# Validation-m3sSAGE/GCN_Recommendation

Measured on AMD Instinct MI355X. Metric: propagated edges/sec (SpMM) + Recall@20, Amazon-Books 3-layer d=64, higher is better.
Workload: dtype f32; 1 GPU; C3 full Amazon-Books-2023 shape (10.3M users x 4.4M items x 29.5M interactions); generator=powerlaw, users=10300000, items=4400000, interactions=29500000, nnz=56305746, d=64, layers=3, brands=0, content_dim=0, hub_threshold=128, hub_mode=exact, emu_min_degree=1024, parallelism=single

## Files before the change

gcn_recommendation_amd/csrc/lgcn_engine.hip:

```cpp
#include "lgcn_kernels.h"

#include <string.h>
#include <algorithm>
#include <functional>
#include <new>
#include <vector>

namespace lgcn_detail {
int g_rows_per_group = 0;
int g_unroll = 0;
int g_mean_prefetch = 0;
int g_min_groups = 0;
int g_emu_margin = (128 << 4) | 4;
int g_sample_blocks = 0;
int g_fusion_bwd_blocks = 0;
}

namespace {
__global__ void k_coo_inspect(const int64_t* __restrict__ rows, const int64_t* __restrict__ cols,
                              int64_t nnz, int32_t n_rows, int32_t n_cols, int32_t* flags) {
    const int64_t j = (int64_t)blockIdx.x * blockDim.x + threadIdx.x;
    if (j >= nnz) return;
    const int64_t r = rows[j], c = cols[j];
    int f = 0;
// ... 964 lines not shown
    if (d < 1 || d > 2048 || n_hub_rows < 0) return LGCN_EINVAL;
    if (n_pre_rows < 0 || n_pre_rows > n_hub_rows) return LGCN_EINVAL;
    if (int e = check_epi(epi_host)) return e;
    if (n_hub_rows > 0 && (!hub_rows || !partials || !y || ldy < d)) return LGCN_EINVAL;
    return hub_combine(hub_rows, n_hub_rows, n_pre_rows, partials, y, ldy, d, *epi_host,
                       S(stream));
}

int lgcn_scale_rows(lgcn_rows_t x, int32_t n_rows, int32_t d, float div, float* y, int64_t ldy,
                    void* stream) {
    if (int e = valid_geom(n_rows, d)) return e;
    if (n_rows > 0 && (!y || ldy < d)) return LGCN_EINVAL;
    return scale_rows(x, n_rows, d, div, y, ldy, S(stream));
}

}

namespace {
constexpr int kPoolEvents = 1024;
struct EventPool {
    hipEvent_t ev[kPoolEvents];
    int n = 0;
    int next = 0;
    int32_t state[5] = {0, 0, 0, 0, 0};
};
struct StreamSet {
    hipStream_t aux[3];
    int n_aux;
};
struct Marks {
    hipEvent_t t0, t1;
    hipEvent_t* trace;
};
}

struct lgcn_sched {
    StreamSet lane0;
    EventPool* pool;
    int32_t slots[2];
    int chain;
    Marks marks;
    hipStream_t lane1_main;
    StreamSet lane1;
    hipEvent_t* trace_sides;
    hipEvent_t* timing_sides;
    int classes;
    int lk_normal;
// ... 57 lines not shown
                           static_cast<char*>(p.emu_meta) + b0 * d * LGCN_EMU_META_BYTES,
                           p.emu_stage ? p.emu_stage + b0 * (d + 1) * LGCN_EMU_BLOCK : nullptr,
                           live, s);
}

int part_walk(const lgcn_edge_t* edges, const lgcn_hub_plan_t& p, const EmuPart& q,
              const lgcn_rows_t& x, float xdiv, const uint32_t* x_nz, float* y, int64_t ldy,
              int32_t d, const lgcn_epilogue_t& ep, int slots, const lgcn_emu_row_t* live,
              hipStream_t s) {
    if (q.r1 <= q.r0) return 0;
    return lgcn_emu_walk(edges, p.emu_blocks, p.emu_rows + q.r0, q.r1 - q.r0, p.emu_rel,
                         p.emu_meta, p.emu_stage, x, xdiv, x_nz, y, ldy, d, &ep, slots,
                         live ? live + q.r0 : nullptr, s);
}

bool chain_ok(const lgcn_rows_t& x, int32_t d) {
    return lgcn_chain_supported(d) && x.ld % 4 == 0 && al16(x.p0) && al16(x.p1) && al16(x.p2);
}

int plan_layer(const int32_t* rowptr, const lgcn_edge_t* edges, const int32_t* row_ids,
               int32_t n, const lgcn_hub_plan_t& p, const lgcn_rows_t& x, float xdiv,
               const uint32_t* x_nz, float* y, int64_t ldy, int32_t d, const lgcn_epilogue_t& ep,
               const lgcn_sched* root, const StreamSet* ss, const Marks& mk, hipStream_t s,
               Deps* dp = nullptr) {
    const lgcn_sched* sc = ss ? root : nullptr;
    const int32_t ne = p.n_emu_rows;
    const bool live = x_nz && p.emu_live && ne > 0 && chain_ok(x, d) && (!sc || sc->chain);
    const bool chains = !live && ne > p.emu_part_rows[1] && chain_ok(x, d) && (!sc || sc->chain);
    if ((chains || live ? p.emu_part_blocks[1] : p.n_emu_blocks) > p.emu_scratch_blocks)
        return LGCN_EINVAL;
    hipEvent_t* tr = mk.trace;
    auto mark = [&](int k, hipStream_t st) -> int {
        return tr && tr[k] ? herr(hipEventRecord(tr[k], st)) : 0;
    };
    const EmuPart parts[3] = {{0, p.emu_part_rows[0], 0, p.emu_part_blocks[0]},
                              {p.emu_part_rows[0], p.emu_part_rows[1], p.emu_part_blocks[0],
                               p.emu_part_blocks[1]},
                              {p.emu_part_rows[1], ne, p.emu_part_blocks[1], p.n_emu_blocks}};
    const int slots[3] = {sc ? sc->slots[0] : 0, sc ? sc->slots[1] : 0, sc ? sc->slots[1] : 0};
    auto layer_kernel = [&](hipStream_t st) -> int {
        if (mk.t0)
            if (int e = herr(hipEventRecord(mk.t0, st))) return e;
        if (int e = spmm_layer(rowptr, edges, row_ids, n, p.threshold, p.items, p.n_items,
                               p.partials, x, y, ldy, d, ep, xdiv, x_nz, st))
            return e;
        if (mk.t1)
            if (int e = herr(hipEventRecord(mk.t1, st))) return e;
        return hub_combine(p.rows, p.n_rows, p.n_pre, p.partials, y, ldy, d, ep, st);
    };
    const bool has_late = dp && (dp->late[0] || dp->late[1] || dp->late[2] ||
                                 dp->late_emu[0] || dp->late_emu[1]);
    const bool defer_epi = sc && has_late && ep.mode == LGCN_EPI_MEAN && p.emu_out && ne > 0 &&
                           !live;
    lgcn_epilogue_t ep_rows;
    memset(&ep_rows, 0, sizeof(ep_rows));
    ep_rows.mode = LGCN_EPI_ROWS;
    auto emu_y = [&](int i) { return defer_epi ? p.emu_out + (int64_t)parts[i].r0 * d : y; };
    const int64_t emu_ld = defer_epi ? d : ldy;
    const lgcn_epilogue_t& emu_ep = defer_epi ? ep_rows : ep;
    auto chain_rows = [&](hipStream_t st) -> int {
        const EmuPart& q = parts[2];
        if (q.r1 <= q.r0) return 0;
        return lgcn_chain_rows(edges, p.emu_blocks, p.emu_rows + q.r0, q.r1 - q.r0, x, xdiv,
                               emu_y(2), emu_ld, d, &emu_ep, st);
    };
    const lgcn_emu_row_t* lflags =
        live ? lgcn_live_flags(p.emu_live, ne, p.n_emu_blocks) : nullptr;
    auto live_rows = [&](hipStream_t st) -> int {
        return lgcn_live_rows(edges, p.emu_blocks, p.n_emu_blocks, p.emu_rows, ne, x, xdiv, x_nz,
                              y, ldy, d, &ep, p.emu_part_rows[1], LGCN_LIVE_MAX, p.emu_live, st);
    };
    auto walked = [&](int i, hipStream_t st) -> int {
        if (int e = part_blocks(edges, p, parts[i], x, xdiv, x_nz, d, lflags, st)) return e;
        return part_walk(edges, p, parts[i], x, xdiv, x_nz, y, ldy, d, ep, slots[i], lflags, st);
    };
    auto done_on_s = [&]() -> int {
        if (dp && dp->defer && sc)
            for (int i = 0; i < 2; ++i)
                if (int e = record(sc, s, &dp->part_done[i])) return e;
        return 0;
    };
    if (!sc || ne == 0 || live) {
        if (int e = wait_late(s, dp)) return e;
    }
    if (live && sc) {
        const int na = ss->n_aux;
// ... 16 lines not shown
        if (int e = mark(5, a0)) return e;
        if (int e = walked(1, a1)) return e;
        if (int e = mark(6, a1)) return e;
        if (int e = layer_kernel(s)) return e;
        if (int e = mark(3, s)) return e;
        if (int e = link(sc, a0, s)) return e;
        if (a1 != a0)
            if (int e = link(sc, a1, s)) return e;
        if (a2 != a0 && a2 != a1)
            if (int e = link(sc, a2, s)) return e;
        if (int e = mark(7, s)) return e;
        return done_on_s();
    }
    if (live) {
        if (int e = live_rows(s)) return e;
        for (int i = 0; i < 2; ++i)
            if (int e = walked(i, s)) return e;
        if (int e = layer_kernel(s)) return e;
        return done_on_s();
    }
    if (!sc || ne == 0) {
        for (int i = 0; i < 3; ++i)
            if (i < 2 || !chains)
                if (int e = part_blocks(edges, p, parts[i], x, xdiv, x_nz, d, nullptr, s)) return e;
        if (int e = layer_kernel(s)) return e;
        for (int i = 0; i < 3; ++i)
            if (i < 2 || !chains)
                if (int e = part_walk(edges, p, parts[i], x, xdiv, x_nz, y, ldy, d, ep, slots[i],
                                      nullptr, s))
                    return e;
        if (chains)
            if (int e = chain_rows(s)) return e;
        return done_on_s();
    }
    const int na = ss->n_aux;
    const bool own = dp && na >= 3;
    auto aux_of = [&](int part) { return ss->aux[part < na ? part : na - 1]; };
    if (int e = mark(0, s)) return e;
    hipEvent_t fork;
    if (int e = record(sc, s, &fork)) return e;
    for (int i = 0; i < na; ++i) {
        const hipEvent_t w = own && i < 2 && dp->part_wait[i] ? dp->part_wait[i] : fork;
        if (int e = wait_ev(ss->aux[i], w)) return e;
    }
    for (int i = 0; i < 3; ++i)
        if (i < 2 || !chains) {
            if (int e = part_blocks(edges, p, parts[i], x, xdiv, x_nz, d, nullptr, aux_of(i)))
                return e;
            if (i < 2)
                if (int e = mark(1 + i, aux_of(i))) return e;
        }
    if (int e = wait_late(s, dp, !defer_epi)) return e;
    if (!defer_epi)
        for (int i = 0; i < na; ++i)
            if (int e = wait_late(ss->aux[i], dp)) return e;
    if (parts[0].b1 > parts[0].b0)
        if (int e = link(sc, aux_of(0), s)) return e;
    if (dp && dp->lk && dp->lk != s) {
        if (int e = link(sc, s, dp->lk)) return e;
        if (int e = layer_kernel(dp->lk)) return e;
        if (int e = link(sc, dp->lk, s)) return e;
    } else if (int e = layer_kernel(s)) {
        return e;
    }
    if (int e = mark(3, s)) return e;
    if (chains) {
        if (int e = chain_rows(aux_of(2))) return e;
        if (int e = mark(4, aux_of(2))) return e;
    }
    for (int i = 0; i < 3; ++i)
        if (i < 2 || !chains) {
            if (int e = part_walk(edges, p, parts[i], x, xdiv, x_nz, emu_y(i), emu_ld, d, emu_ep,
                                  slots[i], nullptr, aux_of(i)))
                return e;
            if (i < 2)
                if (int e = mark(5 + i, aux_of(i))) return e;
        }
    for (int i = 0; i < na; ++i) {
        if (own && dp->defer && i < 2) {
            if (int e = record(sc, ss->aux[i], &dp->part_done[i])) return e;
        } else if (int e = link(sc, ss->aux[i], s)) {
            return e;
        }
    }
    if (defer_epi) {
        for (hipEvent_t e : dp->late_emu)
            if (int r = wait_ev(s, e)) return r;
        if (int e = lgcn_emu_epilogue(p.emu_rows, ne, p.emu_out, d, y, ldy, d, &ep, s)) return e;
    }
    if (int e = mark(7, s)) return e;
    return own ? 0 : done_on_s();
}

struct Lane {
    hipStream_t main;
// ... 149 lines not shown

int run_layers(const int32_t* rowptr, const lgcn_edge_t* edges, const int32_t* row_ids, int32_t n,
               const lgcn_hub_plan_t* plan, int32_t d, int32_t K,
               const std::function<LayerIO(int)>& layer, void* const* ev_host,
               const lgcn_sched* sched, hipStream_t s) {
    if (int e = check_plan(plan)) return e;
    if (sched) sched->pool->next = 0;
    for (int k = 1; k <= K; ++k) {
        const LayerIO io = layer(k);
        if (ev_host)
            if (int e = herr(hipEventRecord((hipEvent_t)ev_host[2 * (k - 1)], s))) return e;
        if (int e = plan_layer(rowptr, edges, row_ids, n, *plan, io.x, io.xdiv, io.x_nz, io.y, d, d,
                               io.ep, sched, sched ? &sched->lane0 : nullptr,
                               sched ? sched->marks : Marks{}, s))
            return e;
        if (ev_host)
            if (int e = herr(hipEventRecord((hipEvent_t)ev_host[2 * (k - 1) + 1], s))) return e;
    }
    return 0;
}

int seg_layer(const int32_t* rowptr, const lgcn_edge_t* edges, const lgcn_shared_t& sr,
              int32_t lo, int32_t hi, const lgcn_hub_plan_t* plans, int k, int g,
              const LayerIO& io, int32_t d, const lgcn_sched* sc, const Lane& L, Deps* dp) {
    const int32_t* row_ids = sr.row_ids;
    const int32_t empty_tail = sr.empty_tail[g], shared_tail = sr.shared_tail[g];
    const int32_t* rep = sr.rep;
    for (int j = 0; j < g; ++j) rep += sr.shared_tail[j];
    if (empty_tail > 0) {
        hi -= empty_tail;
        if (io.ep.mode == LGCN_EPI_MEAN)
            if (int e = mean_empty(row_ids + hi, empty_tail, io.ep, io.y, d, d, L.main)) return e;
    }
    hi -= shared_tail;
    const bool has_shared = shared_tail > 0 && io.ep.mode == LGCN_EPI_MEAN;
    auto shared_mean = [&](hipStream_t st) -> int {
        if (!has_shared) return 0;
        return mean_shared(rowptr + hi, edges, row_ids + hi, rep, shared_tail, io.x, io.ep, io.y,
                           d, d, st);
    };
    hipStream_t side = nullptr;
    if (has_shared && hi > lo && L.ss && L.ss->n_aux > 0 && !capture_restricted(L.main)) {
        side = L.ss->aux[L.ss->n_aux > 1 ? 1 : 0];
        if (int e = link(sc, L.main, side)) return e;
        if (int e = wait_late(side, dp)) return e;
        if (int e = shared_mean(side)) return e;
    }
    if (hi <= lo) {
        if (dp && dp->defer && sc)
            for (int i = 0; i < 2; ++i)
                if (int e = record(sc, L.main, &dp->part_done[i])) return e;
        if (has_shared)
            if (int e = wait_late(L.main, dp)) return e;
        return shared_mean(L.main);
    }
    const int h = (k - 1) * kSegs + g;
    Marks mk{};
    if (L.ss) {
        mk.t0 = sc->timing_sides ? sc->timing_sides[2 * h] : nullptr;
        mk.t1 = sc->timing_sides ? sc->timing_sides[2 * h + 1] : nullptr;
        mk.trace = sc->trace_sides ? sc->trace_sides + h * 8 : nullptr;
    }
    Deps local;
    Deps* dq = dp;
    if (!L.ss && dp && dp->defer && sc) {
        local = *dp;
        local.defer = false;
        dq = &local;
    }
    if (int e = plan_layer(rowptr + lo, edges, row_ids + lo, hi - lo, plans[2 * g + (k & 1)],
                           io.x, io.xdiv, io.x_nz, io.y, d, d, io.ep, sc, L.ss, mk, L.main, dq))
        return e;
    if (dq == &local)
        for (int i = 0; i < 2; ++i)
            if (int e = record(sc, L.main, &dp->part_done[i])) return e;
    if (side) return link(sc, side, L.main);
    return shared_mean(L.main);
}

int run_sides(const int32_t* rowptr, const lgcn_shared_t& sr, const lgcn_sides_t& sd,
              const lgcn_hub_plan_t* plans, int32_t d, int32_t K,
              const std::function<LayerIO(int)>& layer, const lgcn_sched* sched, hipStream_t s) {
    Lane lanes[2];
    bool l1_aux = false;
    if (sched) sched->pool->next = 0;
    const bool two = make_lanes(sched, s, lanes, l1_aux);
    const bool cap = capture_restricted(s);
    const bool classes = sched && sched->classes && classes_hold(sd, plans) && !cap;
    if (sched) sched->pool->state[3] = classes ? 1 : 0;
    const int32_t lo[kSegs] = {0, sd.class_end[0], sd.class_end[1], sd.split};
    const int32_t hi[kSegs] = {sd.class_end[0], sd.class_end[1], sd.split, 0};
    auto seg_hi = [&](int g, int32_t n) { return g == 3 ? n : hi[g]; };
    const int32_t n = sd.n;
    if (int e = fork_lanes(sched, two, lanes[1], s)) return e;
    constexpr int KM = LGCN_MAX_LAYERS + 2;
    hipEvent_t cls[KM][3] = {}, ab[KM] = {}, rest[KM] = {}, part[KM][2] = {};
    for (int k = 1; k <= K; ++k) {
        const LayerIO io = layer(k);
        const bool mean = io.ep.mode == LGCN_EPI_MEAN;
        {
            const Lane& L = lanes[(k + 1 + K) & 1];
            Deps dp;
            if (classes && k >= 2) {
                dp.part_wait[0] = cls[k - 1][0];
                dp.part_wait[1] = ab[k - 1];
            }
            dp.defer = k < K && sched && !cap;
            if (k == K && mean && sched && sched->lk_normal && two && l1_aux && !cap &&
                sched->lane0.n_aux >= 3)
                dp.lk = sched->lane0.aux[2];
            if (mean && k >= 2) {
                dp.late[0] = rest[k - 1];
                dp.late_emu[0] = part[k - 1][0];
                dp.late_emu[1] = part[k - 1][1];
            }
            if (int e = seg_layer(rowptr, k >= 2 ? sr.edges_ln : sr.edges_l1, sr, sd.split, n,
                                  plans, k, 3, io, d, sched, L, &dp))
                return e;
            if (k < K && sched) {
                if (int e = record(sched, L.main, &rest[k])) return e;
                part[k][0] = dp.part_done[0];
                part[k][1] = dp.part_done[1];
            }
        }
        {
            const Lane& L = lanes[(k + K) & 1];
            static const int up[3] = {0, 1, 2}, down[3] = {2, 1, 0};
            const int* order = k == 1 ? up : down;
            for (int t = 0; t < 3; ++t) {
                const int c = order[t];
                if (k >= 2 && (c <= 1 || !classes))
                    if (int e = wait_ev(L.main, part[k - 1][1])) return e;
                if (k >= 2 && (c == 0 || !classes))
                    if (int e = wait_ev(L.main, part[k - 1][0])) return e;
                Deps dp;
                if (mean && k >= 2) dp.late[0] = cls[k - 1][c];
                if (int e = seg_layer(rowptr, sr.edges_l1, sr, lo[c], seg_hi(c, n), plans, k, c,
                                      io, d, sched, L, &dp))
                    return e;
                if (sched)
                    if (int e = record(sched, L.main, &cls[k][c])) return e;
            }
            ab[k] = k == 1 ? cls[k][1] : cls[k][0];
        }
    }
    return join_lanes(sched, two, lanes[1], s);
}
lgcn_shared_t plain_rows(const int32_t* row_ids, const lgcn_edge_t* edges,
                         const int32_t* empty_tail) {
    lgcn_shared_t sr;
    memset(&sr, 0, sizeof(sr));
    sr.row_ids = row_ids;
    sr.edges_l1 = sr.edges_ln = edges;
    if (empty_tail) memcpy(sr.empty_tail, empty_tail, sizeof(sr.empty_tail));
    return sr;
}

int forward_sides(const int32_t* rowptr, const lgcn_sides_t* sides, const lgcn_hub_plan_t* plans,
                  const lgcn_shared_t& in, bool ptrs_ok, const lgcn_rows_t& emb, int32_t d,
                  int32_t K, float* const* layer_bufs_host, float* out, const lgcn_sched* sched,
                  void* stream) {
    const int32_t n = sides ? sides->n : -1;
    hipStream_t s = S(stream);
    int rc;
    if (prologue(n, d, K, out && ptrs_ok, layer_bufs_host, emb, out, true, s, &rc)) return rc;
    if (int e = check_sides(rowptr, in.row_ids, n, sides, plans)) return e;
    const int32_t b[kSegs + 1] = {0, sides->class_end[0], sides->class_end[1], sides->split, n};
    bool any = false;
    for (int g = 0; g < kSegs; ++g) {
        const int32_t et = in.empty_tail[g], st = in.shared_tail[g];
        if (et < 0 || st < 0 || (int64_t)et + st > b[g + 1] - b[g]) return LGCN_EINVAL;
        any = any || st > 0;
    }
    if (in.shared_tail[3] != 0) return LGCN_EINVAL;
    if ((in.shared_tail[0] > 0) + (in.shared_tail[1] > 0) + (in.shared_tail[2] > 0) > 1)
        return LGCN_EINVAL;
    if (any && (!in.row_ids || !in.edges_l1 || !in.edges_ln || !in.rep)) return LGCN_EINVAL;
    const lgcn_shared_t sr =
        K >= 2 && any ? in : plain_rows(in.row_ids, in.edges_l1, in.empty_tail);
    auto layer = [&](int k) { return forward_io(k, K, emb, layer_bufs_host, out, n, d); };
    return run_sides(rowptr, sr, *sides, plans, d, K, layer, sched, s);
}
}

extern "C" {

int lgcn_sched_create(void* const* aux_streams, int32_t n_aux, lgcn_sched_t** out) {
    if (!out || n_aux < 1 || n_aux > 7 || !aux_streams) return LGCN_EINVAL;
    for (int i = 0; i < n_aux; ++i)
        if (!aux_streams[i]) return LGCN_EINVAL;
    lgcn_sched* sc = new (std::nothrow) lgcn_sched();
    EventPool* pool = new (std::nothrow) EventPool();
    if (!sc || !pool) {
        delete sc;
        delete pool;
        return LGCN_EINVAL;
    }
    memset(sc, 0, sizeof(*sc));
    sc->pool = pool;
    const int n0 = n_aux < 3 ? n_aux : 3;
    sc->lane0.n_aux = sc->lane0_rev.n_aux = n0;
    sc->chain = 1;
    sc->classes = 1;
    sc->lk_normal = 1;
// ... 52 lines not shown
        case LGCN_SCHED_TRACE:
            sc->marks.trace = reinterpret_cast<hipEvent_t*>(value);
            return 0;
        case LGCN_SCHED_TRACE_SIDES:
            sc->trace_sides = reinterpret_cast<hipEvent_t*>(value);
            return 0;
        case LGCN_SCHED_TIMING_SIDES:
            sc->timing_sides = reinterpret_cast<hipEvent_t*>(value);
            return 0;
        case LGCN_SCHED_CLASSES:
            sc->classes = value != 0;
            return 0;
        case LGCN_SCHED_LK_NORMAL:
            sc->lk_normal = value != 0;
            return 0;
        default:
            return LGCN_EINVAL;
    }
}

int lgcn_capture_full_schedule(void) { return runtime_captures_full() ? 1 : 0; }

int64_t lgcn_sched_state(const lgcn_sched_t* sc, int32_t what) {
    if (!sc || what < LGCN_SCHED_STATE_LANES || what > LGCN_SCHED_STATE_CAPTURE_FULL)
        return LGCN_EINVAL;
    return sc->pool->state[what - LGCN_SCHED_STATE_LANES];
}

int lgcn_layer(const int32_t* rowptr, const lgcn_edge_t* edges, const int32_t* row_ids,
               int32_t n_rows, const lgcn_hub_plan_t* plan, lgcn_rows_t x, float x_div,
               const uint32_t* x_nz, float* y, int64_t ldy, int32_t d,
               const lgcn_epilogue_t* epi_host, const lgcn_sched_t* sched, void* stream) {
    if (int e = valid_geom(n_rows, d)) return e;
    if (int e = check_epi(epi_host)) return e;
    if (int e = check_plan(plan)) return e;
    if (n_rows > 0 && (!rowptr || !y || ldy < d)) return LGCN_EINVAL;
    if (!(x_div > 0.f)) return LGCN_EINVAL;
    if (epi_host->mode != LGCN_EPI_ADD && (x_div != 1.f || x_nz)) return LGCN_EINVAL;
    if (sched) sched->pool->next = 0;
    return plan_layer(rowptr, edges, row_ids, n_rows, *plan, x, x_div, x_nz, y, ldy, d,
                      *epi_host, sched, sched ? &sched->lane0 : nullptr,
                      sched ? sched->marks : Marks{}, S(stream));
}

int lgcn_propagate_forward(const int32_t* rowptr, const lgcn_edge_t* edges,
                           const int32_t* row_ids, int32_t n, const lgcn_hub_plan_t* plan,
                           lgcn_rows_t emb, int32_t d,
// ... 73 lines not shown
```

gcn_recommendation_amd/csrc/lgcn_exact.hip:

```cpp
#include <hip/hip_runtime.h>
#include <stdint.h>
#include <string.h>

#include <algorithm>
#include <atomic>

#include "lgcn.h"

namespace lgcn_detail {
extern int g_emu_margin;
int live_prepare(const lgcn_edge_t* edges, const lgcn_emu_block_t* blocks, int32_t n_blocks,
                 const lgcn_emu_row_t* rows, int32_t n_rows, const uint32_t* x_nz, int32_t d,
                 float x_div, const lgcn_epilogue_t* epi_host, float* y, int64_t ldy,
                 const void* x_p0, int32_t live_min, int32_t max_live, void* scratch,
                 hipStream_t s);
int live_chains(int32_t n_blocks, int32_t n_rows, lgcn_rows_t x, float x_div, float* y,
                int64_t ldy, int32_t d, const lgcn_epilogue_t* epi_host, void* scratch,
                hipStream_t s);
}

namespace {

constexpr int kNB = LGCN_EMU_CANDS;
constexpr int kEOff = 2;
constexpr int kSlack = 132;
constexpr int kLB = (1 << 23) + kSlack;
constexpr int kHB = (1 << 24) - kSlack;
constexpr int kC = 3 << 22;
// ... 5 lines not shown
#endif
#if LGCN_ROWMAJOR
#define LGCN_GRID_COL(nc) (blockIdx.x % (uint32_t)(nc))
#define LGCN_GRID_ROW(nc) (blockIdx.x / (uint32_t)(nc))
#define LGCN_GRID_DIM(cols, rows) dim3((cols) * (rows))
#else
#define LGCN_GRID_COL(nc) blockIdx.y
#define LGCN_GRID_ROW(nc) blockIdx.x
#define LGCN_GRID_DIM(cols, rows) dim3((rows), (cols))
#endif
static_assert(LGCN_EMU_META_BYTES == 16, "meta record is one int4");


__device__ __forceinline__ const float* seg_row_x(const lgcn_rows_t& s, int32_t r) {
    if (r < s.end0) return s.p0 + (int64_t)r * s.ld;
    if (r < s.end1) return s.p1 + (int64_t)(r - s.end0) * s.ld;
    return s.p2 + (int64_t)(r - s.end1) * s.ld;
}

__device__ __forceinline__ bool row_live_x(const uint32_t* __restrict__ nz, int32_t r) {
    return (nz[r >> 5] >> (r & 31)) & 1u;
}

__device__ __forceinline__ const float* seg_row_sel(const lgcn_rows_t& s, int32_t r) {
    const char* b = reinterpret_cast<const char*>(s.p0);
    const int64_t row_b = s.ld * 4;
    const int64_t d1 = (reinterpret_cast<const char*>(s.p1) - b) - (int64_t)s.end0 * row_b;
    const int64_t d2 = (reinterpret_cast<const char*>(s.p2) - b) - (int64_t)s.end1 * row_b;
    const int64_t off = (int64_t)r * row_b + (r < s.end0 ? 0 : (r < s.end1 ? d1 : d2));
    return reinterpret_cast<const float*>(b + off);
}

template <int XD>
__device__ __forceinline__ float load_elem(const lgcn_rows_t& x, const uint32_t* x_nz, int32_t col,
                                           int c, float xdiv, bool ok = true) {
    float v = *reinterpret_cast<const float*>(
        reinterpret_cast<const char*>(seg_row_sel(x, col)) + (uint32_t)c * 4u);
    if constexpr ((XD & 4) != 0) ok = ok && row_live_x(x_nz, col);
    v = ok ? v : 0.f;
    if constexpr ((XD & 3) == 1) return v / xdiv;
    else if constexpr ((XD & 3) == 2) return v * xdiv;
    else return v;
}

__device__ __forceinline__ int lsb_exp(float f) {
    const uint32_t b = __float_as_uint(f);
    const int E = (int)((b >> 23) & 255u);
    return __builtin_ctz(b | 0x800000u) + max(E, 1) - 150;
}

__device__ __forceinline__ int lsb_exp_z(float f) {
    return (__float_as_uint(f) << 1) ? lsb_exp(f) : -100000;
}


#if defined(LGCN_EMU_STATS) || defined(LGCN_EMU_MODES)
__device__ int g_blk_mode;
#define LGCN_BLK_OFF(b) ((blk_mode & (b)) != 0)
#else
#define LGCN_BLK_OFF(b) false
#endif
template <int XD>
__global__ __launch_bounds__(64) void k_emu_blocks(const lgcn_edge_t* __restrict__ edges,
                                                   const lgcn_emu_block_t* __restrict__ blocks,
                                                   lgcn_rows_t x, float xdiv,
                                                   const uint32_t* __restrict__ x_nz, int32_t d,
                                                   int4* __restrict__ ktab,
                                                   int4* __restrict__ meta,
                                                   float* __restrict__ stage,
                                                   const lgcn_emu_row_t* __restrict__ live) {
#ifndef LGCN_BLK_SW
#define LGCN_BLK_SW 16
#endif
    constexpr int SW = LGCN_BLK_SW;
    static_assert(SW == 8 || SW == 16, "sub-window");
    const int lane = threadIdx.x;
    const int c = blockIdx.y * 64 + lane;
    const bool act = c < d;
    const int64_t bi = blockIdx.x;
    const lgcn_emu_block_t blk = blocks[bi];
    if (live && live[blk.row].n_blocks) return;
#if defined(LGCN_EMU_STATS) || defined(LGCN_EMU_MODES)
    const int blk_mode = __builtin_amdgcn_readfirstlane(g_blk_mode);
#endif
    float T = 0.f, tlo = 0.f, thi = 0.f;
    int maxlsb = -100000;
    float cand[kNB];
    bool init = false;
    int ebase = 0;
    const int cc = act ? c : d - 1;
    auto load_rec = [&](int32_t j0) {
        const int32_t j = min(j0 + lane, blk.end - 1);
        const int2 r = *reinterpret_cast<const int2*>(edges + j);
        return j0 + lane < blk.end ? r : make_int2(0, 0);
    };
    auto load_sub = [&](const int2& rec, int s0, int n, float (&xv)[SW], float (&vv)[SW]) {
#pragma unroll
        for (int t = 0; t < SW; ++t) {
            const int32_t col = __builtin_amdgcn_readlane(rec.x, s0 + t);
            vv[t] = __int_as_float(__builtin_amdgcn_readlane(rec.y, s0 + t));
            xv[t] = load_elem<XD>(x, x_nz, col, cc, xdiv, act && s0 + t < n);
        }
    };
    constexpr int TP = 36;
    __shared__ __attribute__((aligned(16))) float s_tile[64 * TP];
    float* const st0 = stage ? stage + bi * (d + 1) * LGCN_EMU_BLOCK : nullptr;
    float* sv = stage && blockIdx.y == 0 ? stage + (bi * (d + 1) + d) * LGCN_EMU_BLOCK : nullptr;
    const bool staging = st0 && !LGCN_BLK_OFF(1);
    auto stage_sub = [&](const float (&xv)[SW], int part) {
        if (!staging) return;
        float* tp = s_tile + lane * TP + SW * part;
#pragma unroll
        for (int q = 0; q < SW / 4; ++q)
            *reinterpret_cast<float4*>(tp + 4 * q) =
                make_float4(xv[4 * q], xv[4 * q + 1], xv[4 * q + 2], xv[4 * q + 3]);
    };
    auto wave_sync = [] {
        __builtin_amdgcn_fence(__ATOMIC_RELEASE, "wavefront");
        __builtin_amdgcn_wave_barrier();
        __builtin_amdgcn_fence(__ATOMIC_ACQUIRE, "wavefront");
    };
    auto stage_flush = [&](int step0) {
        if (!staging) return;
        wave_sync();
        const int sub = lane >> 3, q = lane & 7;
#pragma unroll
        for (int i = 0; i < 8; ++i) {
            const int col = 8 * i + sub;
            const float4 v = *reinterpret_cast<const float4*>(s_tile + col * TP + 4 * q);
            const int cg = blockIdx.y * 64 + col;
            if (cg < d) {
                typedef float f4v __attribute__((ext_vector_type(4)));
                __builtin_nontemporal_store(
                    f4v{v.x, v.y, v.z, v.w},
                    reinterpret_cast<f4v*>(st0 + (int64_t)cg * LGCN_EMU_BLOCK + step0 + 4 * q));
            }
        }
        wave_sync();
    };
    auto run_sub = [&](const float (&xv)[SW], const float (&vv)[SW]) {
        if (!init) {
            float s = T, m = 0.f;
#pragma unroll
            for (int t = 0; t < SW; ++t) {
                s = __builtin_fmaf(vv[t], xv[t], s);
                m = fmaxf(m, fabsf(s));
            }
            if (m > 0.f && m <= 3.0e38f) {
                init = true;
                int e;
                frexpf(m, &e);
                ebase = max(-200, min(e - 1 + kEOff + 1, 200));
#pragma unroll
                for (int k = 0; k < kNB; ++k) {
                    const int eb = ebase + k;
                    cand[k] = (eb >= -126 && eb <= 127) ? ldexpf(1.5f, eb) : 1.5f;
                }
            }
        }
#pragma unroll
        for (int t = 0; t < SW; ++t) {
            T = __builtin_fmaf(vv[t], xv[t], T);
            tlo = fminf(tlo, T);
            thi = fmaxf(thi, T);
            if (!LGCN_BLK_OFF(4)) maxlsb = max(maxlsb, lsb_exp_z(vv[t]) + lsb_exp_z(xv[t]));
        }
        if (init && !LGCN_BLK_OFF(2)) {
#pragma unroll
            for (int t = 0; t < SW; ++t) {
#pragma unroll
                for (int k = 0; k < kNB; ++k) cand[k] = __builtin_fmaf(vv[t], xv[t], cand[k]);
            }
        }
    };
    int2 rec = load_rec(blk.beg);
    float xa[SW], va[SW], xb[SW], vb[SW];
    load_sub(rec, 0, min(64, blk.end - blk.beg), xa, va);
    for (int32_t j0 = blk.beg; j0 < blk.end; j0 += 64) {
        const int n = min(64, blk.end - j0);
        const bool more = j0 + 64 < blk.end;
        const int2 nrec = load_rec(j0 + 64);
        if (sv) sv[j0 - blk.beg + lane] = __int_as_float(rec.y);
        const int w0 = j0 - blk.beg;
#pragma unroll
        for (int k = 0; k < 64 / SW; k += 2) {
            load_sub(rec, (k + 1) * SW, n, xb, vb);
            run_sub(xa, va);
            stage_sub(xa, k % (32 / SW));
            if (k + 2 < 64 / SW)
                load_sub(rec, (k + 2) * SW, n, xa, va);
            else if (more)
                load_sub(nrec, 0, min(64, blk.end - j0 - 64), xa, va);
            run_sub(xb, vb);
            stage_sub(xb, (k + 1) % (32 / SW));
            if ((k + 2) % (32 / SW) == 0) stage_flush(w0 + (k + 2 - 32 / SW) * SW);
        }
        rec = nrec;
    }
    if (!act) return;
    const int64_t rc = bi * d + c;
    const float M = fmaxf(-tlo, thi);
    double err = 0.0;
    if (M > 0.f) {
        int e;
        frexpf(M, &e);
        err = (LGCN_EMU_BLOCK / 2) * ldexp(1.0, max(e - 24, -149));
    }
    const double lo_u = floor(ldexp((double)tlo - err, 23 - ebase));
    const double hi_u = ceil(ldexp((double)thi + err, 23 - ebase));
    const bool fits = lo_u >= -1073741824.0 && hi_u <= 1073741824.0;
    const int32_t lo0 = fits ? (int32_t)lo_u : 0, hi0 = fits ? (int32_t)hi_u : 0;
    uint32_t vm = 0;
    int K[kNB];
#pragma unroll
    for (int k = 0; k < kNB; ++k) {
        const int eb = ebase + k;
        const bool normal = eb >= -126 && eb <= 127;
        const float a0 = normal ? ldexpf(1.5f, eb) : 1.5f;
        const float ku = ldexpf(cand[k] - a0, 23 - eb);
        const bool kfit = fabsf(ku) < 16777216.f;
        K[k] = (init && kfit) ? (int)ku : 0;
// ... 508 lines not shown
        s = s + out;
        out = ep.pad ? s * __int_as_float(ep.pad) : s / ep.div;
    } else if constexpr (MODE == LGCN_EPI_ADD) {
        if (!ep.addend_nz || row_live_x(ep.addend_nz, row)) {
            const float z = seg_row_x(ep.addend, row)[c];
            out = (ep.pad ? z * __int_as_float(ep.pad) : z / ep.div) + out;
        }
    }
    y[(int64_t)row * ldy + c] = out;
}

inline int herr_x(hipError_t e) { return e == hipSuccess ? 0 : (int)e; }

bool is_pow2(float x) {
    int e;
    return x > 0.f && frexpf(x, &e) == 0.5f;
}

template <int XD>
int launch_blocks(const lgcn_edge_t* edges, const lgcn_emu_block_t* blocks, int32_t n_blocks,
                  const lgcn_rows_t& x, float xdiv, const uint32_t* x_nz, int32_t d, int4* ktab,
                  int4* meta, float* stage, const lgcn_emu_row_t* live, hipStream_t s) {
    const dim3 grid((uint32_t)n_blocks, (uint32_t)((d + 63) / 64));
    hipLaunchKernelGGL((k_emu_blocks<XD>), grid, dim3(64), 0, s, edges, blocks, x, xdiv, x_nz, d,
                       ktab, meta, stage, live);
    return herr_x(hipGetLastError());
}

template <int MODE, int XD>
int launch_walk(const lgcn_edge_t* edges, const lgcn_emu_block_t* blocks,
                const lgcn_emu_row_t* rows, int32_t n_rows, const int4* ktab, const int4* meta,
                const float* stage, const lgcn_rows_t& x, float xdiv, const uint32_t* x_nz, float* y,
                int64_t ldy, int32_t d, const lgcn_epilogue_t& ep, int slots,
                const lgcn_emu_row_t* live, hipStream_t s) {
    const dim3 grid = LGCN_GRID_DIM((uint32_t)d, (uint32_t)n_rows);
    const size_t lds = (size_t)(2 * slots + 1) * 2 * LGCN_EMU_BLOCK * sizeof(float);
    if (lds > 56 * 1024) {
        static std::atomic<uint64_t> raised{0};
        int dev = 0;
        if (hipError_t e = hipGetDevice(&dev)) return (int)e;
        const uint64_t bit = dev < 64 ? (1ull << dev) : 0;
        if (!bit || !(raised.load(std::memory_order_relaxed) & bit)) {
            const hipError_t e = hipFuncSetAttribute(
                reinterpret_cast<const void*>(&k_emu_walk<MODE, XD>),
                hipFuncAttributeMaxDynamicSharedMemorySize, 160 * 1024 - 8 * 1024);
            if (e != hipSuccess) return (int)e;
            raised.fetch_or(bit, std::memory_order_relaxed);
        }
// ... 600 lines not shown
```

gcn_recommendation_amd/engine.py:

```python
import ctypes
import os
import threading

import numpy as np
import torch

_PKG = os.path.dirname(os.path.abspath(__file__))
LIB_PATH = os.path.join(_PKG, "liblgcn_engine.so")

LGCN_EPI_STORE, LGCN_EPI_MEAN, LGCN_EPI_ADD = 0, 1, 2
LGCN_SCATTER_STORE, LGCN_SCATTER_ADD = 0, 1
LGCN_MAX_LAYERS = 16
COO_ROWS_UNSORTED, COO_OUT_OF_RANGE, COO_COLS_UNSORTED = 1, 2, 4
INT32_MAX = 2 ** 31 - 1
TUNE_ROWS_PER_GROUP, TUNE_UNROLL, TUNE_MEAN_PREFETCH, TUNE_MIN_GROUPS = 1, 2, 3, 4
TUNE_EMU_MARGIN = 6
TUNE_SAMPLE_BLOCKS = 7
TUNE_FUSION_BWD_BLOCKS = 8
FUSION_BWD_CHUNK = 2048
SCHED_SLOTS0, SCHED_SLOTS1, SCHED_CHAIN, SCHED_TIMING_START, SCHED_TIMING_END, SCHED_TRACE = \
    1, 2, 3, 4, 5, 6
SCHED_TRACE_SIDES, SCHED_TIMING_SIDES = 7, 8
SCHED_CLASSES = 16
SCHED_LK_NORMAL = 17
SCHED_LANE1_SHARED = 18
SCHED_STATE_LANES, SCHED_STATE_L1_AUX, SCHED_STATE_CAPTURING, SCHED_STATE_CLASSES = 1, 2, 3, 4
SCHED_STATE_CAPTURE_FULL = 5
N_SEGS = 4
TRACE_PHASES = ("start", "part0_blocks", "part1_blocks", "layer_kernel", "chain_rows",
                "part0_walk", "part1_walk", "joined")
ABI_VERSION = 14
LGCN_EMU_CANDS, LGCN_EMU_META_BYTES, LGCN_EMU_BLOCK = 16, 16, 256
ADAM_MAX_TENSORS, ADAM_CHUNK = 16, 4096
BPR_MAX_NEG = 64

DEFAULT_HUB_THRESHOLD = 128
HUB_MODES = ("exact", "chunk")


def hub_mode_from_env():
    m = os.environ.get("LGCN_HUB_MODE", "exact").lower()
    if m not in HUB_MODES:
        raise LgcnError(f"LGCN_HUB_MODE={m!r} ({' | '.join(HUB_MODES)})")
    return m


def emu_defer_enabled():
    return os.environ.get("LGCN_EMU_DEFER", "1") != "0"


# ... 1209 lines not shown
        if self.sc is not None:
            self.sc.set(SCHED_TIMING_SIDES, 0)
            self.sc.set(SCHED_TRACE_SIDES, 0)


side_trace = None
side_timing = None


last_schedule = None


def _note_schedule(sc, graph):
    global last_schedule
    if sc is None:
        last_schedule = {"sided": True, "aux_streams": 0, "lanes": 1, "lane1_aux": 0,
                         "captured": torch.cuda.is_current_stream_capturing(), "classes": False}
        return
    last_schedule = {"sided": True, "aux_streams": sc.n_aux,
                     "lanes": sc.state(SCHED_STATE_LANES),
                     "lane1_aux": sc.state(SCHED_STATE_L1_AUX),
                     "captured": bool(sc.state(SCHED_STATE_CAPTURING)),
                     "capture_full": bool(sc.state(SCHED_STATE_CAPTURE_FULL)),
                     "classes": bool(sc.state(SCHED_STATE_CLASSES))}


def use_sides(graph, layer_events=None, kernel_events=None):
    return graph.split is not None and layer_events is None and kernel_events is None


def _collect_sides(ev, K, graph):
    segs = [g for g, (a, b) in enumerate(graph.segments()) if b > a]
    if ev.timing is not None and side_timing is not None:
        side_timing.append({(k, g): (ev.timing[((k - 1) * N_SEGS + g) * 2],
                                     ev.timing[((k - 1) * N_SEGS + g) * 2 + 1])
                            for k in range(1, K + 1) for g in segs})
    if ev.trace is not None and side_trace is not None:
        side_trace.append({(k, g): list(zip(TRACE_PHASES,
                                            ev.trace[((k - 1) * N_SEGS + g) * 8:
                                                     ((k - 1) * N_SEGS + g + 1) * 8]))
                           for k in range(1, K + 1) for g in segs})


def _run_sided(what, call, sc, K, graph):
    ev = _SideEvents(sc, K, side_timing is not None, side_trace is not None)
    try:
        _check(call(sc.handle if sc is not None else None), what)
# ... 307 lines not shown
```

include/lgcn.h:

```cpp
#ifndef LGCN_H_
#define LGCN_H_

#include <stdint.h>
#include <stddef.h>

#ifdef __cplusplus
extern "C" {
#endif

#define LGCN_ABI_VERSION 14

#define LGCN_EINVAL      (-1)
#define LGCN_EALIGN      (-2)
#define LGCN_ETOOMANY    (-3)

#define LGCN_MAX_LAYERS 16

#define LGCN_COO_ROWS_UNSORTED   1
#define LGCN_COO_OUT_OF_RANGE    2
#define LGCN_COO_COLS_UNSORTED   4

#define LGCN_EPI_STORE 0
#define LGCN_EPI_MEAN  1
#define LGCN_EPI_ADD   2
// ... 201 lines not shown
const lgcn_emu_row_t* lgcn_live_flags(const void* scratch, int32_t n_rows, int32_t n_blocks);

typedef struct lgcn_sched lgcn_sched_t;
int lgcn_sched_create(void* const* aux_streams, int32_t n_aux, lgcn_sched_t** out);
int lgcn_sched_destroy(lgcn_sched_t* sched);
#define LGCN_SCHED_SLOTS0        1
#define LGCN_SCHED_SLOTS1        2
#define LGCN_SCHED_CHAIN         3
#define LGCN_SCHED_TIMING_START  4
#define LGCN_SCHED_TIMING_END    5
#define LGCN_SCHED_TRACE         6
#define LGCN_SCHED_TRACE_SIDES   7
#define LGCN_SCHED_TIMING_SIDES  8
#define LGCN_SCHED_CLASSES      16
#define LGCN_SCHED_LK_NORMAL    17
#define LGCN_SCHED_LANE1_SHARED 18
int lgcn_capture_full_schedule(void);
int lgcn_sched_set(lgcn_sched_t* sched, int32_t knob, int64_t value);
#define LGCN_SCHED_STATE_LANES     1
#define LGCN_SCHED_STATE_L1_AUX    2
#define LGCN_SCHED_STATE_CAPTURING 3
#define LGCN_SCHED_STATE_CLASSES   4
#define LGCN_SCHED_STATE_CAPTURE_FULL 5
int64_t lgcn_sched_state(const lgcn_sched_t* sched, int32_t what);

int lgcn_layer(const int32_t* rowptr, const lgcn_edge_t* edges, const int32_t* row_ids,
               int32_t n_rows, const lgcn_hub_plan_t* plan, lgcn_rows_t x, float x_div,
               const uint32_t* x_nz, float* y, int64_t ldy, int32_t d,
               const lgcn_epilogue_t* epi_host, const lgcn_sched_t* sched, void* stream);

int lgcn_propagate_forward(const int32_t* rowptr, const lgcn_edge_t* edges,
                           const int32_t* row_ids, int32_t n, const lgcn_hub_plan_t* plan,
                           lgcn_rows_t emb, int32_t d,
                           int32_t K, float* const* layer_bufs_host, float* out,
                           void* const* ev_host, const lgcn_sched_t* sched, void* stream);

int lgcn_propagate_backward(const int32_t* rowptr, const lgcn_edge_t* edges,
                            const int32_t* row_ids, int32_t n, const lgcn_hub_plan_t* plan,
                            lgcn_rows_t grad_out,
                            const uint32_t* grad_nz, int32_t d, int32_t K, float* work_h,
                            float* grad_e0, const lgcn_sched_t* sched, void* stream);

typedef struct {
    int32_t n;
    int32_t split;
    int32_t class_end[2];
// ... 181 lines not shown
```

Before: 14.79 billion edges/s.

## Use single-buffer view for layer-1 emulated rows and precompute gather addresses

In the first forward layer, each side's emulated-row kernels get a single-buffer view of the segmented input when the needed rows lie in one buffer. This lets k_emu_blocks use a SEG1 specialization with plain row*stride addressing. The kernel also moves per-edge address computation, LSB exponents and live masks into the per-window record load, broadcasting them with readlane instead of recomputing per element. It adds a full-window specialization that skips tail masking. The intent is to cut the integer and select overhead on the gather path, at the cost of more template variants and pointer arithmetic that assumes one contiguous buffer.

```diff
diff --git a/gcn_recommendation_amd/csrc/lgcn_engine.hip b/gcn_recommendation_amd/csrc/lgcn_engine.hip
--- a/gcn_recommendation_amd/csrc/lgcn_engine.hip
+++ b/gcn_recommendation_amd/csrc/lgcn_engine.hip
@@ -1010,7 +1010,7 @@
     hipEvent_t ev[kPoolEvents];
     int n = 0;
     int next = 0;
-    int32_t state[5] = {0, 0, 0, 0, 0};
+    int32_t state[6] = {0, 0, 0, 0, 0, 0};
 };
 struct StreamSet {
     hipStream_t aux[3];
@@ -1114,11 +1114,12 @@
                int32_t n, const lgcn_hub_plan_t& p, const lgcn_rows_t& x, float xdiv,
                const uint32_t* x_nz, float* y, int64_t ldy, int32_t d, const lgcn_epilogue_t& ep,
                const lgcn_sched* root, const StreamSet* ss, const Marks& mk, hipStream_t s,
-               Deps* dp = nullptr) {
+               Deps* dp = nullptr, const lgcn_rows_t* x_emu = nullptr) {
     const lgcn_sched* sc = ss ? root : nullptr;
+    const lgcn_rows_t& xw = x_emu ? *x_emu : x;
     const int32_t ne = p.n_emu_rows;
     const bool live = x_nz && p.emu_live && ne > 0 && chain_ok(x, d) && (!sc || sc->chain);
-    const bool chains = !live && ne > p.emu_part_rows[1] && chain_ok(x, d) && (!sc || sc->chain);
+    const bool chains = !live && ne > p.emu_part_rows[1] && chain_ok(xw, d) && (!sc || sc->chain);
     if ((chains || live ? p.emu_part_blocks[1] : p.n_emu_blocks) > p.emu_scratch_blocks)
         return LGCN_EINVAL;
     hipEvent_t* tr = mk.trace;
@@ -1153,7 +1154,7 @@
     auto chain_rows = [&](hipStream_t st) -> int {
         const EmuPart& q = parts[2];
         if (q.r1 <= q.r0) return 0;
-        return lgcn_chain_rows(edges, p.emu_blocks, p.emu_rows + q.r0, q.r1 - q.r0, x, xdiv,
+        return lgcn_chain_rows(edges, p.emu_blocks, p.emu_rows + q.r0, q.r1 - q.r0, xw, xdiv,
                                emu_y(2), emu_ld, d, &emu_ep, st);
     };
     const lgcn_emu_row_t* lflags =
@@ -1216,11 +1217,11 @@
     if (!sc || ne == 0) {
         for (int i = 0; i < 3; ++i)
             if (i < 2 || !chains)
-                if (int e = part_blocks(edges, p, parts[i], x, xdiv, x_nz, d, nullptr, s)) return e;
+                if (int e = part_blocks(edges, p, parts[i], xw, xdiv, x_nz, d, nullptr, s)) return e;
         if (int e = layer_kernel(s)) return e;
         for (int i = 0; i < 3; ++i)
             if (i < 2 || !chains)
-                if (int e = part_walk(edges, p, parts[i], x, xdiv, x_nz, y, ldy, d, ep, slots[i],
+                if (int e = part_walk(edges, p, parts[i], xw, xdiv, x_nz, y, ldy, d, ep, slots[i],
                                       nullptr, s))
                     return e;
         if (chains)
@@ -1239,7 +1240,7 @@
     }
     for (int i = 0; i < 3; ++i)
         if (i < 2 || !chains) {
-            if (int e = part_blocks(edges, p, parts[i], x, xdiv, x_nz, d, nullptr, aux_of(i)))
+            if (int e = part_blocks(edges, p, parts[i], xw, xdiv, x_nz, d, nullptr, aux_of(i)))
                 return e;
             if (i < 2)
                 if (int e = mark(1 + i, aux_of(i))) return e;
@@ -1264,7 +1265,7 @@
     }
     for (int i = 0; i < 3; ++i)
         if (i < 2 || !chains) {
-            if (int e = part_walk(edges, p, parts[i], x, xdiv, x_nz, emu_y(i), emu_ld, d, emu_ep,
+            if (int e = part_walk(edges, p, parts[i], xw, xdiv, x_nz, emu_y(i), emu_ld, d, emu_ep,
                                   slots[i], nullptr, aux_of(i)))
                 return e;
             if (i < 2)
@@ -1460,7 +1461,8 @@
 
 int seg_layer(const int32_t* rowptr, const lgcn_edge_t* edges, const lgcn_shared_t& sr,
               int32_t lo, int32_t hi, const lgcn_hub_plan_t* plans, int k, int g,
-              const LayerIO& io, int32_t d, const lgcn_sched* sc, const Lane& L, Deps* dp) {
+              const LayerIO& io, int32_t d, const lgcn_sched* sc, const Lane& L, Deps* dp,
+              const lgcn_rows_t* x_emu = nullptr) {
     const int32_t* row_ids = sr.row_ids;
     const int32_t empty_tail = sr.empty_tail[g], shared_tail = sr.shared_tail[g];
     const int32_t* rep = sr.rep;
@@ -1507,7 +1509,8 @@
         dq = &local;
     }
     if (int e = plan_layer(rowptr + lo, edges, row_ids + lo, hi - lo, plans[2 * g + (k & 1)],
-                           io.x, io.xdiv, io.x_nz, io.y, d, d, io.ep, sc, L.ss, mk, L.main, dq))
+                           io.x, io.xdiv, io.x_nz, io.y, d, d, io.ep, sc, L.ss, mk, L.main, dq,
+                           x_emu))
         return e;
     if (dq == &local)
         for (int i = 0; i < 2; ++i)
@@ -1516,9 +1519,32 @@
     return shared_mean(L.main);
 }
 
+bool one_buffer_view(const lgcn_rows_t& x, const lgcn_sides_t& sd, int side, lgcn_rows_t* v) {
+    if (x.p0 == x.p1 && x.p1 == x.p2) return false;
+    const int32_t n = sd.n;
+    if (x.end0 < 0 || x.end0 > x.end1 || x.end1 > n || x.end1 - x.end0 != n - sd.split)
+        return false;
+    const float* p;
+    int32_t first;
+    if (side == 0) {
+        p = x.p1, first = x.end0;
+    } else if (x.end1 == n) {
+        p = x.p0, first = 0;
+    } else if (x.end0 == 0) {
+        p = x.p2, first = x.end1;
+    } else {
+        return false;
+    }
+    if (!p) return false;
+    const uintptr_t b = reinterpret_cast<uintptr_t>(p) - (uintptr_t)first * (uintptr_t)x.ld * 4u;
+    *v = dense_rows(reinterpret_cast<const float*>(b), n, x.ld);
+    return true;
+}
+
 int run_sides(const int32_t* rowptr, const lgcn_shared_t& sr, const lgcn_sides_t& sd,
               const lgcn_hub_plan_t* plans, int32_t d, int32_t K,
-              const std::function<LayerIO(int)>& layer, const lgcn_sched* sched, hipStream_t s) {
+              const std::function<LayerIO(int)>& layer, const lgcn_sched* sched, hipStream_t s,
+              bool l1_view = false) {
     Lane lanes[2];
     bool l1_aux = false;
     if (sched) sched->pool->next = 0;
@@ -1536,6 +1562,12 @@
     for (int k = 1; k <= K; ++k) {
         const LayerIO io = layer(k);
         const bool mean = io.ep.mode == LGCN_EPI_MEAN;
+        lgcn_rows_t view[2];
+        const lgcn_rows_t* xe[2] = {nullptr, nullptr};
+        if (l1_view && k == 1)
+            for (int sdx = 0; sdx < 2; ++sdx)
+                if (one_buffer_view(io.x, sd, sdx, &view[sdx])) xe[sdx] = &view[sdx];
+        if (sched && k == 1) sched->pool->state[5] = (xe[1] ? 1 : 0) | (xe[0] ? 2 : 0);
         {
             const Lane& L = lanes[(k + 1 + K) & 1];
             Deps dp;
@@ -1553,7 +1585,7 @@
                 dp.late_emu[1] = part[k - 1][1];
             }
             if (int e = seg_layer(rowptr, k >= 2 ? sr.edges_ln : sr.edges_l1, sr, sd.split, n,
-                                  plans, k, 3, io, d, sched, L, &dp))
+                                  plans, k, 3, io, d, sched, L, &dp, xe[1]))
                 return e;
             if (k < K && sched) {
                 if (int e = record(sched, L.main, &rest[k])) return e;
@@ -1574,7 +1606,7 @@
                 Deps dp;
                 if (mean && k >= 2) dp.late[0] = cls[k - 1][c];
                 if (int e = seg_layer(rowptr, sr.edges_l1, sr, lo[c], seg_hi(c, n), plans, k, c,
-                                      io, d, sched, L, &dp))
+                                      io, d, sched, L, &dp, xe[0]))
                     return e;
                 if (sched)
                     if (int e = record(sched, L.main, &cls[k][c])) return e;
@@ -1617,7 +1649,7 @@
     const lgcn_shared_t sr =
         K >= 2 && any ? in : plain_rows(in.row_ids, in.edges_l1, in.empty_tail);
     auto layer = [&](int k) { return forward_io(k, K, emb, layer_bufs_host, out, n, d); };
-    return run_sides(rowptr, sr, *sides, plans, d, K, layer, sched, s);
+    return run_sides(rowptr, sr, *sides, plans, d, K, layer, sched, s, true);
 }
 }
 
@@ -1716,7 +1748,7 @@
 int lgcn_capture_full_schedule(void) { return runtime_captures_full() ? 1 : 0; }
 
 int64_t lgcn_sched_state(const lgcn_sched_t* sc, int32_t what) {
-    if (!sc || what < LGCN_SCHED_STATE_LANES || what > LGCN_SCHED_STATE_CAPTURE_FULL)
+    if (!sc || what < LGCN_SCHED_STATE_LANES || what > LGCN_SCHED_STATE_L1_VIEW)
         return LGCN_EINVAL;
     return sc->pool->state[what - LGCN_SCHED_STATE_LANES];
 }
diff --git a/gcn_recommendation_amd/csrc/lgcn_exact.hip b/gcn_recommendation_amd/csrc/lgcn_exact.hip
--- a/gcn_recommendation_amd/csrc/lgcn_exact.hip
+++ b/gcn_recommendation_amd/csrc/lgcn_exact.hip
@@ -4,6 +4,7 @@
 
 #include <algorithm>
 #include <atomic>
+#include <type_traits>
 
 #include "lgcn.h"
 
@@ -55,13 +56,15 @@
     return (nz[r >> 5] >> (r & 31)) & 1u;
 }
 
-__device__ __forceinline__ const float* seg_row_sel(const lgcn_rows_t& s, int32_t r) {
+__device__ __forceinline__ int64_t seg_row_off(const lgcn_rows_t& s, int32_t r) {
     const char* b = reinterpret_cast<const char*>(s.p0);
     const int64_t row_b = s.ld * 4;
     const int64_t d1 = (reinterpret_cast<const char*>(s.p1) - b) - (int64_t)s.end0 * row_b;
     const int64_t d2 = (reinterpret_cast<const char*>(s.p2) - b) - (int64_t)s.end1 * row_b;
-    const int64_t off = (int64_t)r * row_b + (r < s.end0 ? 0 : (r < s.end1 ? d1 : d2));
-    return reinterpret_cast<const float*>(b + off);
+    return (int64_t)r * row_b + (r < s.end0 ? 0 : (r < s.end1 ? d1 : d2));
+}
+__device__ __forceinline__ const float* seg_row_sel(const lgcn_rows_t& s, int32_t r) {
+    return reinterpret_cast<const float*>(reinterpret_cast<const char*>(s.p0) + seg_row_off(s, r));
 }
 
 template <int XD>
@@ -93,7 +96,7 @@
 #else
 #define LGCN_BLK_OFF(b) false
 #endif
-template <int XD>
+template <int XD, bool SEG1>
 __global__ __launch_bounds__(64) void k_emu_blocks(const lgcn_edge_t* __restrict__ edges,
                                                    const lgcn_emu_block_t* __restrict__ blocks,
                                                    lgcn_rows_t x, float xdiv,
@@ -118,21 +121,49 @@
 #endif
     float T = 0.f, tlo = 0.f, thi = 0.f;
     int maxlsb = -100000;
-    float cand[kNB];
+    float cand[kNB] = {};
     bool init = false;
     int ebase = 0;
     const int cc = act ? c : d - 1;
+    struct Rec {
+        int2 r;
+        uint64_t a;
+        int vl;
+        uint64_t lm;
+    };
+    const uint64_t x0 = reinterpret_cast<uint64_t>(x.p0);
+    const uint32_t row_b = (uint32_t)(x.ld * 4);
     auto load_rec = [&](int32_t j0) {
         const int32_t j = min(j0 + lane, blk.end - 1);
         const int2 r = *reinterpret_cast<const int2*>(edges + j);
-        return j0 + lane < blk.end ? r : make_int2(0, 0);
-    };
-    auto load_sub = [&](const int2& rec, int s0, int n, float (&xv)[SW], float (&vv)[SW]) {
+        Rec o;
+        if constexpr (SEG1) o.a = x0 + (uint64_t)(uint32_t)r.x * row_b;
+        else o.a = x0 + (uint64_t)seg_row_off(x, r.x);
+        o.r = j0 + lane < blk.end ? r : make_int2(0, 0);
+        o.vl = lsb_exp_z(__int_as_float(o.r.y));
+        if constexpr ((XD & 4) != 0) o.lm = __ballot(row_live_x(x_nz, o.r.x));
+        else o.lm = 0;
+        return o;
+    };
+    auto load_sub = [&](auto full, const Rec& rec, int s0, int n, float (&xv)[SW]) {
+        constexpr bool FULL = decltype(full)::value;
+        typedef const __attribute__((address_space(1))) char* gptr;
+        uint32_t co = (uint32_t)cc * 4u;
+        asm volatile("" : "+v"(co));
 #pragma unroll
         for (int t = 0; t < SW; ++t) {
-            const int32_t col = __builtin_amdgcn_readlane(rec.x, s0 + t);
-            vv[t] = __int_as_float(__builtin_amdgcn_readlane(rec.y, s0 + t));
-            xv[t] = load_elem<XD>(x, x_nz, col, cc, xdiv, act && s0 + t < n);
+            const uint32_t lo = (uint32_t)__builtin_amdgcn_readlane((int)(uint32_t)rec.a, s0 + t);
+            const uint32_t hi = (uint32_t)__builtin_amdgcn_readlane((int)(rec.a >> 32), s0 + t);
+            float v = *reinterpret_cast<const __attribute__((address_space(1))) float*>(
+                reinterpret_cast<gptr>(((uint64_t)hi << 32) | lo) + co);
+            if constexpr (!FULL || (XD & 4) != 0) {
+                uint32_t keep = FULL ? ~0u : (uint32_t)((s0 + t - n) >> 31);
+                if constexpr ((XD & 4) != 0) keep &= 0u - (uint32_t)((rec.lm >> (s0 + t)) & 1u);
+                v = __uint_as_float(__float_as_uint(v) & keep);
+            }
+            if constexpr ((XD & 3) == 1) v = v / xdiv;
+            else if constexpr ((XD & 3) == 2) v = v * xdiv;
+            xv[t] = v;
         }
     };
     constexpr int TP = 36;
@@ -157,12 +188,14 @@
         if (!staging) return;
         wave_sync();
         const int sub = lane >> 3, q = lane & 7;
+        int dd = d;
+        asm volatile("" : "+s"(dd));
 #pragma unroll
         for (int i = 0; i < 8; ++i) {
             const int col = 8 * i + sub;
             const float4 v = *reinterpret_cast<const float4*>(s_tile + col * TP + 4 * q);
             const int cg = blockIdx.y * 64 + col;
-            if (cg < d) {
+            if (cg < dd) {
                 typedef float f4v __attribute__((ext_vector_type(4)));
                 __builtin_nontemporal_store(
                     f4v{v.x, v.y, v.z, v.w},
@@ -171,7 +204,11 @@
         }
         wave_sync();
     };
-    auto run_sub = [&](const float (&xv)[SW], const float (&vv)[SW]) {
+    auto run_sub = [&](const float (&xv)[SW], const Rec& rec, int s0) {
+        float vv[SW];
+#pragma unroll
+        for (int t = 0; t < SW; ++t)
+            vv[t] = __int_as_float(__builtin_amdgcn_readlane(rec.r.y, s0 + t));
         if (!init) {
             float s = T, m = 0.f;
 #pragma unroll
@@ -196,9 +233,10 @@
             T = __builtin_fmaf(vv[t], xv[t], T);
             tlo = fminf(tlo, T);
             thi = fmaxf(thi, T);
-            if (!LGCN_BLK_OFF(4)) maxlsb = max(maxlsb, lsb_exp_z(vv[t]) + lsb_exp_z(xv[t]));
-        }
-        if (init && !LGCN_BLK_OFF(2)) {
+            if (!LGCN_BLK_OFF(4))
+                maxlsb = max(maxlsb, __builtin_amdgcn_readlane(rec.vl, s0 + t) + lsb_exp_z(xv[t]));
+        }
+        if (!LGCN_BLK_OFF(2)) {
 #pragma unroll
             for (int t = 0; t < SW; ++t) {
 #pragma unroll
@@ -206,30 +244,34 @@
             }
         }
     };
-    int2 rec = load_rec(blk.beg);
-    float xa[SW], va[SW], xb[SW], vb[SW];
-    load_sub(rec, 0, min(64, blk.end - blk.beg), xa, va);
-    for (int32_t j0 = blk.beg; j0 < blk.end; j0 += 64) {
-        const int n = min(64, blk.end - j0);
-        const bool more = j0 + 64 < blk.end;
-        const int2 nrec = load_rec(j0 + 64);
-        if (sv) sv[j0 - blk.beg + lane] = __int_as_float(rec.y);
-        const int w0 = j0 - blk.beg;
-#pragma unroll
-        for (int k = 0; k < 64 / SW; k += 2) {
-            load_sub(rec, (k + 1) * SW, n, xb, vb);
-            run_sub(xa, va);
-            stage_sub(xa, k % (32 / SW));
-            if (k + 2 < 64 / SW)
-                load_sub(rec, (k + 2) * SW, n, xa, va);
-            else if (more)
-                load_sub(nrec, 0, min(64, blk.end - j0 - 64), xa, va);
-            run_sub(xb, vb);
-            stage_sub(xb, (k + 1) % (32 / SW));
-            if ((k + 2) % (32 / SW) == 0) stage_flush(w0 + (k + 2 - 32 / SW) * SW);
-        }
-        rec = nrec;
-    }
+    auto windows = [&](auto full) {
+        Rec rec = load_rec(blk.beg);
+        float xa[SW], xb[SW];
+        load_sub(full, rec, 0, min(64, blk.end - blk.beg), xa);
+        for (int32_t j0 = blk.beg; j0 < blk.end; j0 += 64) {
+            const int n = min(64, blk.end - j0);
+            const bool more = j0 + 64 < blk.end;
+            const Rec nrec = load_rec(j0 + 64);
+            if (sv) sv[j0 - blk.beg + lane] = __int_as_float(rec.r.y);
+            const int w0 = j0 - blk.beg;
+#pragma unroll
+            for (int k = 0; k < 64 / SW; k += 2) {
+                load_sub(full, rec, (k + 1) * SW, n, xb);
+                run_sub(xa, rec, k * SW);
+                stage_sub(xa, k % (32 / SW));
+                if (k + 2 < 64 / SW)
+                    load_sub(full, rec, (k + 2) * SW, n, xa);
+                else if (more)
+                    load_sub(full, nrec, 0, min(64, blk.end - j0 - 64), xa);
+                run_sub(xb, rec, (k + 1) * SW);
+                stage_sub(xb, (k + 1) % (32 / SW));
+                if ((k + 2) % (32 / SW) == 0) stage_flush(w0 + (k + 2 - 32 / SW) * SW);
+            }
+            rec = nrec;
+        }
+    };
+    if (blk.end - blk.beg == LGCN_EMU_BLOCK) windows(std::true_type{});
+    else windows(std::false_type{});
     if (!act) return;
     const int64_t rc = bi * d + c;
     const float M = fmaxf(-tlo, thi);
@@ -784,8 +826,13 @@
                   const lgcn_rows_t& x, float xdiv, const uint32_t* x_nz, int32_t d, int4* ktab,
                   int4* meta, float* stage, const lgcn_emu_row_t* live, hipStream_t s) {
     const dim3 grid((uint32_t)n_blocks, (uint32_t)((d + 63) / 64));
-    hipLaunchKernelGGL((k_emu_blocks<XD>), grid, dim3(64), 0, s, edges, blocks, x, xdiv, x_nz, d,
-                       ktab, meta, stage, live);
+    const bool seg1 = x.p0 == x.p1 && x.p1 == x.p2 && x.ld >= 0 && x.ld * 4 <= (int64_t)UINT32_MAX;
+    if (seg1)
+        hipLaunchKernelGGL((k_emu_blocks<XD, true>), grid, dim3(64), 0, s, edges, blocks, x, xdiv,
+                           x_nz, d, ktab, meta, stage, live);
+    else
+        hipLaunchKernelGGL((k_emu_blocks<XD, false>), grid, dim3(64), 0, s, edges, blocks, x, xdiv,
+                           x_nz, d, ktab, meta, stage, live);
     return herr_x(hipGetLastError());
 }
 
diff --git a/gcn_recommendation_amd/engine.py b/gcn_recommendation_amd/engine.py
--- a/gcn_recommendation_amd/engine.py
+++ b/gcn_recommendation_amd/engine.py
@@ -26,6 +26,7 @@
 SCHED_LANE1_SHARED = 18
 SCHED_STATE_LANES, SCHED_STATE_L1_AUX, SCHED_STATE_CAPTURING, SCHED_STATE_CLASSES = 1, 2, 3, 4
 SCHED_STATE_CAPTURE_FULL = 5
+SCHED_STATE_L1_VIEW = 6
 N_SEGS = 4
 TRACE_PHASES = ("start", "part0_blocks", "part1_blocks", "layer_kernel", "chain_rows",
                 "part0_walk", "part1_walk", "joined")
@@ -1281,7 +1282,8 @@
                      "lane1_aux": sc.state(SCHED_STATE_L1_AUX),
                      "captured": bool(sc.state(SCHED_STATE_CAPTURING)),
                      "capture_full": bool(sc.state(SCHED_STATE_CAPTURE_FULL)),
-                     "classes": bool(sc.state(SCHED_STATE_CLASSES))}
+                     "classes": bool(sc.state(SCHED_STATE_CLASSES)),
+                     "l1_view": sc.state(SCHED_STATE_L1_VIEW)}
 
 
 def use_sides(graph, layer_events=None, kernel_events=None):
diff --git a/include/lgcn.h b/include/lgcn.h
--- a/include/lgcn.h
+++ b/include/lgcn.h
@@ -247,6 +247,7 @@
 #define LGCN_SCHED_STATE_CAPTURING 3
 #define LGCN_SCHED_STATE_CLASSES   4
 #define LGCN_SCHED_STATE_CAPTURE_FULL 5
+#define LGCN_SCHED_STATE_L1_VIEW   6
 int64_t lgcn_sched_state(const lgcn_sched_t* sched, int32_t what);
 
 int lgcn_layer(const int32_t* rowptr, const lgcn_edge_t* edges, const int32_t* row_ids,
```

Result: no change. 14.68 billion edges/s (-0.7%).
